# VictoriaMetrics/VictoriaLogs

Hardware: AMD Instinct MI355X
Metric: matched-rows/sec (higher is better)
Workload: dtype u8; 1 GPU; 100M rows, AND(phrase, re2 regex) on two string columns, 1xMI355X; rows_per_gpu=100000000, live_rows_per_gpu=100000000, msg_len=256, matched_rows_per_pass=100000000, parallelism=dp1

## Files before the change

### victorialogs_amd/csrc/core/regex.cpp

```cpp
#include "regex.h"

#include <cstring>

#include "match.h"
#include "tokenizer.h"
#include "unicode_case.h"

namespace vl {

namespace {

struct RNode {
  enum Kind {
    Lit, Dot, Concat, Alt, Star, Plus, Quest, Group, Empty, Class, Assert
  } kind;
  std::string lit;
  std::vector<RNode> subs;
  uint8_t cls[32] = {0};
  bool cls_nonascii = false;
  uint8_t assert_kind = 0;
};

static const uint32_t kFoldOrbits[][4] = {
    {0x004B, 0x006B, 0x212A, 0},
// ... 534 lines not shown
        out.push_back("");
        return true;
      }
      std::vector<std::string> prefixes;
      if (!get_or_values(n.subs[0], prefixes) || prefixes.empty()) return false;
      if (n.subs.size() == 1) {
        out = std::move(prefixes);
        return true;
      }
      RNode rest;
      rest.kind = RNode::Concat;
      rest.subs.assign(n.subs.begin() + 1, n.subs.end());
      std::vector<std::string> suffixes;
      if (!get_or_values(rest, suffixes) || suffixes.empty()) return false;
      if (prefixes.size() * suffixes.size() > kMaxOrValues) return false;
      for (const auto& p : prefixes) {
        for (const auto& q : suffixes) out.push_back(p + q);
      }
      return true;
    }
    default:
      return false;
  }
}

void collect_literals(const RNode& raw, std::vector<std::string>& out) {
  const RNode* n = &raw;
  while (n->kind == RNode::Group) n = &n->subs[0];
  if (n->kind == RNode::Lit) {
    out.push_back(n->lit);
    return;
  }
  if (n->kind != RNode::Concat) return;
  for (const auto& sub : n->subs) {
    const RNode* s = &sub;
    while (s->kind == RNode::Group) s = &s->subs[0];
    if (s->kind == RNode::Lit) out.push_back(s->lit);
  }
}



struct GAtom {
  uint8_t set[32];
};

struct PMask {
  uint64_t w0 = 0, w1 = 0;
  void set(int i) { (i < 64 ? w0 : w1) |= uint64_t(1) << (i & 63); }
  void operator|=(const PMask& o) {
    w0 |= o.w0;
    w1 |= o.w1;
  }
};

template <typename F>
static void pm_foreach(const PMask& m, F f) {
  uint64_t v = m.w0;
  while (v) {
    f(__builtin_ctzll(v));
    v &= v - 1;
  }
  v = m.w1;
  while (v) {
    f(64 + __builtin_ctzll(v));
    v &= v - 1;
  }
// ... 647 lines not shown
```

### victorialogs_amd/csrc/hip/scan_kernels.hip

```cpp
#include <hip/hip_runtime.h>

#include "../core/parse_float.h"
#include "../core/ryu.h"
#include "scan_types.h"

namespace vl {



__device__ int64_t g_vl_local_tz_nsecs = 0;

#include "scan_rowops.h"

typedef const __attribute__((address_space(3))) uint8_t* LdsBytePtr;

struct LdsTileAcc {
  LdsBytePtr tile;
  typedef const __attribute__((address_space(3))) uint64_t* LdsU64Ptr;
  __device__ __forceinline__ long swz(long off) const {
    return TileAcc{nullptr}.swz(off);
  }
  __device__ __forceinline__ uint64_t u64a(long off) const {
    return *(LdsU64Ptr)(tile + swz(off));
  }
  __device__ __forceinline__ void u64a2(long off, uint64_t* x0,
                                        uint64_t* x1) const {
    LdsU64Ptr p = (LdsU64Ptr)(tile + swz(off));
    *x0 = p[0];
    *x1 = p[1];
  }
  __device__ __forceinline__ uint8_t u8(long off) const { return tile[swz(off)]; }
};

__device__ __forceinline__ void d_fill_operand_slot(uint8_t* slot,
                                                    const uint8_t* src,
                                                    uint32_t n, int tid,
                                                    int bdim) {
  for (uint32_t k = tid; k < n; k += bdim) slot[k] = src[k];
}

extern "C" int vql_set_local_tz_nsecs(long long v) {
  int64_t x = v;
  return hipMemcpyToSymbol(HIP_SYMBOL(g_vl_local_tz_nsecs), &x, sizeof(x)) ==
                 hipSuccess
             ? 0
             : -1;
}
// ... 292 lines not shown
      o_next = col_offs[min(r0 + next_wd * 64 + uint32_t(lane), r1)];
      if (lane == 0) o_end_next = col_offs[min(r0 + next_wd * 64 + 64, r1)];
    }
    if (use_tile) {
      asm volatile("s_waitcnt lgkmcnt(0)" ::: "memory");
    }
    bool pred1 = false, pred2 = false;
    if (uint32_t(lane) < ng) {
      const long s = o_lane;
      const long e = uint32_t(__shfl(int(o_lane), lane + 1, 64));
      const long e_fix = uint32_t(lane) == ng - 1 ? long(byte1) : e;
      if (use_tile) {
        LdsTileAcc a{(LdsBytePtr)wtile};
        pred1 = d_match_phrase_at(a, s - byte0, e_fix - s, p1, n1, f1);
        pred2 = d_match_phrase_at(a, s - byte0, e_fix - s, p2, n2, f2);
      } else {
        GlobalAcc a{col_data};
        pred1 = d_match_phrase_at(a, s, e_fix - s, p1, n1, f1);
        pred2 = d_match_phrase_at(a, s, e_fix - s, p2, n2, f2);
      }
    }
    const uint64_t word1 = __ballot(pred1);
    const uint64_t word2 = __ballot(pred2);
    if (lane == 0) {
      out1[wd] = word1;
      out2[wd] = word2;
    }
    o_lane = o_next;
    o_end = o_end_next;
    wd = next_wd;
  }
}

__device__ __forceinline__ bool d_bloom_gate_ok(const DevLeafBlock& lb,
                                                int tid, int bdim,
                                                int* shared_flag) {
  if (!lb.nhashes) return true;
  __syncthreads();
  if (tid == 0) *shared_flag = 1;
  __syncthreads();
  if (lb.bloom_words > 0) {
    const uint64_t max_bits = uint64_t(lb.bloom_words) * 64;
    bool miss = false;
    for (uint32_t k = tid; k < lb.nhashes; k += bdim) {
      uint64_t idx = lb.hashes[k] % max_bits;
      if (((lb.bloom[idx >> 6] >> (idx & 63)) & 1) == 0) miss = true;
    }
    if (miss) *shared_flag = 0;
  }
  __syncthreads();
  return *shared_flag != 0;
}


__global__ __launch_bounds__(256) void scan_program_kernel(
    const DevOp* __restrict__ ops, int nops, const DevLeafBlock* __restrict__ lbs,
    int nleaves, const DevBlock* __restrict__ blocks,
    const DevChunk* __restrict__ chunks, unsigned long long* __restrict__ hits) {
  __shared__ uint64_t stack[kMaxStackDepth][kChunkWords];
  __shared__ __attribute__((aligned(16))) uint8_t tile[kNumWaves * kWaveTileBytes];
  __shared__ int bloom_ok;
  __shared__ unsigned long long wave_sums[4];
  __shared__ __attribute__((aligned(16))) uint8_t opnd[2][kOperandSlotBytes];

  const DevChunk ck = chunks[blockIdx.x];
  const DevBlock blk = blocks[ck.block];
  const uint32_t r0 = ck.chunk * kChunkRows;
  const uint32_t r1 = min(blk.rows, r0 + kChunkRows);
  const uint32_t nwords = (r1 - r0 + 63) / 64;
  const int tid = threadIdx.x;
  const int lane = tid & 63;
  const int wave = tid >> 6;
  const int nwaves = blockDim.x >> 6;
  const LdsBytePtr opnd0 = (LdsBytePtr)&opnd[0][0];
  const LdsBytePtr opnd1 = (LdsBytePtr)&opnd[1][0];

  int sp = 0;
  for (int i = 0; i < nops; i++) {
    const DevOp op = ops[i];
    __syncthreads();
    if (op.kind == kOpLeaf) {
      const DevLeafBlock& lb = lbs[size_t(ck.block) * nleaves + op.leaf];
      uint64_t* out = stack[sp];
      if (i + 1 < nops && ops[i + 1].kind == kOpLeaf &&
          lb.kind == kScanPhraseStr && lb.mode == kModeScan && lb.sg <= 1 &&
          sp + 1 < kMaxStackDepth) {
        const DevLeafBlock& lb2 =
            lbs[size_t(ck.block) * nleaves + ops[i + 1].leaf];
        if (lb2.kind == kScanPhraseStr && lb2.mode == kModeScan &&
            lb2.data == lb.data && lb2.offsets == lb.offsets &&
            lb.operand_len <= kOperandSlotBytes &&
            lb2.operand_len <= kOperandSlotBytes) {
          d_fill_operand_slot(opnd[0], lb.operand, lb.operand_len, tid,
                              blockDim.x);
          d_fill_operand_slot(opnd[1], lb2.operand, lb2.operand_len, tid,
                              blockDim.x);
          const bool ok1 = d_bloom_gate_ok(lb, tid, blockDim.x, &bloom_ok);
          const bool ok2 = d_bloom_gate_ok(lb2, tid, blockDim.x, &bloom_ok);
          __syncthreads();
          if (ok1 && ok2) {
            d_string_phrase2_loop(lb.data, lb.offsets,
                                  tile + wave * kWaveTileBytes, stack[sp],
                                  stack[sp + 1], r0, r1, nwords, lane, wave,
                                  nwaves, opnd0, lb.operand_len, lb.flags,
                                  opnd1, lb2.operand_len, lb2.flags);
            sp += 2;
            i++;
            continue;
          }
        }
      }
      if (lb.mode == kModeNone || lb.mode == kModeAll) {
        uint64_t fill = lb.mode == kModeAll ? ~uint64_t(0) : 0;
        for (uint32_t w = tid; w < nwords; w += blockDim.x) out[w] = fill;
        sp++;
        continue;
      }
      bool lds_phrase = false;
      uint32_t lds_len = 0;
      uint8_t lds_flags = 0;
      if (lb.kind == kScanPhraseStr) {
        if (lb.operand_len <= kOperandSlotBytes) {
          lds_phrase = true;
          lds_len = lb.operand_len;
          lds_flags = lb.flags;
          d_fill_operand_slot(opnd[0], lb.operand, lds_len, tid, blockDim.x);
        }
      } else if (lb.kind == kScanRegexStr) {
        const uint8_t* blob = lb.operand;
        const uint8_t re_flags = blob[0];
        if ((re_flags & kReOnlyPrefix) && !(re_flags & (kReNfa | kReAlways))) {
          const uint32_t plen = uint32_t(blob[1]) | uint32_t(blob[2]) << 8;
          if (plen >= 1 && plen <= kOperandSlotBytes) {
            lds_phrase = true;
            lds_len = plen;
            d_fill_operand_slot(opnd[0], blob + 7, plen, tid, blockDim.x);
          }
        }
      }
      if (!lb.nhashes) {
        if (lds_phrase) __syncthreads();
      } else {
        if (tid == 0) bloom_ok = 1;
        __syncthreads();
        if (lb.bloom_words > 0) {
          const uint64_t max_bits = uint64_t(lb.bloom_words) * 64;
          bool miss = false;
          for (uint32_t k = tid; k < lb.nhashes; k += blockDim.x) {
            uint64_t idx = lb.hashes[k] % max_bits;
            if (((lb.bloom[idx >> 6] >> (idx & 63)) & 1) == 0) miss = true;
          }
          if (miss) bloom_ok = 0;
        }
        __syncthreads();
        if (!bloom_ok) {
          for (uint32_t w = tid; w < nwords; w += blockDim.x) out[w] = 0;
          sp++;
          continue;
        }
      }

      if (d_is_string_kind(lb.kind)) {
        uint8_t* wtile = tile + wave * kWaveTileBytes;
        const uint8_t* col_data = lb.data;
        const uint32_t* col_offs = lb.offsets;
        const uint8_t* op_ptr = lb.operand;
        const uint32_t sgw = lb.sg;
        if (lds_phrase) {
          auto eval = [=](const auto& a, long s0, long sn) {
            return d_match_phrase_at(a, s0, sn, opnd0, lds_len, lds_flags);
          };
          if (sgw > 1) {
            d_string_smallrow_loop<false>(col_data, col_offs, nullptr, nullptr,
                                          wtile, out, r0, r1, nwords, sgw,
                                          lane, wave, nwaves, eval);
          } else {
            d_string_tile_loop<false>(col_data, col_offs, nullptr, nullptr,
                                      wtile, out, r0, r1, nwords, lane, wave,
                                      nwaves, eval);
          }
        } else if (lb.kind == kScanRegexStr) {
          auto eval = [=](const auto& a, long s0, long sn) {
            return d_regex_match_at(op_ptr, a, s0, sn);
          };
          if (sgw > 1) {
            d_string_smallrow_loop<false>(col_data, col_offs, nullptr, nullptr,
                                          wtile, out, r0, r1, nwords, sgw,
                                          lane, wave, nwaves, eval);
          } else {
            d_string_tile_loop<false>(col_data, col_offs, nullptr, nullptr,
                                      wtile, out, r0, r1, nwords, lane, wave,
                                      nwaves, eval);
          }
// ... 345 lines not shown
```

### victorialogs_amd/csrc/hip/scan_rowops.h

```cpp
#pragma once

#include "../core/unicode_ranges.inc"

extern __device__ int64_t g_vl_local_tz_nsecs;

__device__ __forceinline__ bool d_is_token_char(uint8_t c) {
  return (c >= 'a' && c <= 'z') || (c >= 'A' && c <= 'Z') ||
         (c >= '0' && c <= '9') || c == '_';
}

__device__ bool d_is_token_rune(uint32_t r) {
  if (r < 0x80) return d_is_token_char(uint8_t(r));
  int lo = 0, hi = kTokenRuneRangesCount - 1;
  while (lo <= hi) {
    int mid = (lo + hi) >> 1;
    if (r < kTokenRuneRanges[mid][0]) {
      hi = mid - 1;
    } else if (r > kTokenRuneRanges[mid][1]) {
      lo = mid + 1;
    } else {
      return true;
    }
  }
  return false;
// ... 72 lines not shown
  } else if ((c0 & 0xF8) == 0xF0) {
    len = 4; r = c0 & 0x07; lo = 0x10000;
  } else {
    return 0xFFFD;
  }
  if (len > n) return 0xFFFD;
  for (int i = 1; i < len; i++) {
    uint8_t c = a.u8(off + i);
    if ((c & 0xC0) != 0x80) return 0xFFFD;
    r = (r << 6) | (c & 0x3F);
  }
  if (r < lo || r > 0x10FFFF || (r >= 0xD800 && r <= 0xDFFF)) return 0xFFFD;
  *size = len;
  return r;
}

template <typename A>
__device__ uint32_t d_utf8_decode_last(const A& a, long off, long n, int* size) {
  *size = 1;
  if (n <= 0) return 0xFFFD;
  long start = n - 1;
  if (a.u8(off + start) < 0x80) return a.u8(off + start);
  long lim = n >= 4 ? n - 4 : 0;
  while (start > lim && (a.u8(off + start) & 0xC0) == 0x80) start--;
  int sz;
  uint32_t r = d_utf8_decode(a, off + start, n - start, &sz);
  if (start + sz != n) return 0xFFFD;
  *size = sz;
  return r;
}

__device__ __forceinline__ uint64_t d_swar_zero(uint64_t t) {
  return (t - 0x0101010101010101ULL) & ~t & 0x8080808080808080ULL;
}

template <typename A, typename P>
__device__ long d_index_at(const A& a, long s0, long sn, P sub, long subn) {
  if (subn == 0) return 0;
  if (subn > sn) return -1;
  const uint8_t c0 = sub[0];
  const uint64_t pat = 0x0101010101010101ULL * c0;
  const uint64_t pat1 = subn > 1 ? 0x0101010101010101ULL * sub[1] : 0;
  const long last = s0 + sn - subn;
  for (long w = s0 & ~15L; w <= last; w += 32) {
    uint64_t x0, x1, x2, x3;
    a.u64a2(w, &x0, &x1);
    a.u64a2(w + 16, &x2, &x3);
    uint64_t hitA = d_swar_zero(x0 ^ pat);
    uint64_t hitB = d_swar_zero(x1 ^ pat);
    uint64_t hitC = d_swar_zero(x2 ^ pat);
    uint64_t hitD = d_swar_zero(x3 ^ pat);
    if (subn > 1 && (hitA | hitB | hitC | hitD)) {
      const uint64_t h1A = d_swar_zero(x0 ^ pat1);
      const uint64_t h1B = d_swar_zero(x1 ^ pat1);
      const uint64_t h1C = d_swar_zero(x2 ^ pat1);
      const uint64_t h1D = d_swar_zero(x3 ^ pat1);
      hitA &= (h1A >> 8) | ((h1B & 0x80) << 56);
      hitB &= (h1B >> 8) | ((h1C & 0x80) << 56);
      hitC &= (h1C >> 8) | ((h1D & 0x80) << 56);
      hitD &= (h1D >> 8) | 0x8000000000000000ULL;
    }
    if (w < s0) {
      const long off = s0 - w;
      if (off >= 8) {
        hitA = 0;
        hitB &= ~((uint64_t(1) << ((off - 8) * 8)) - 1);
      } else {
        hitA &= ~((uint64_t(1) << (off * 8)) - 1);
      }
    }
    while (hitA | hitB | hitC | hitD) {
      long k;
      if (hitA) {
        k = long(__builtin_ctzll(hitA) >> 3);
        hitA &= hitA - 1;
      } else if (hitB) {
        k = 8 + long(__builtin_ctzll(hitB) >> 3);
        hitB &= hitB - 1;
      } else if (hitC) {
        k = 16 + long(__builtin_ctzll(hitC) >> 3);
        hitC &= hitC - 1;
      } else {
        k = 24 + long(__builtin_ctzll(hitD) >> 3);
        hitD &= hitD - 1;
      }
      const long pos = w + k;
      if (pos > last) return -1;
      bool eq = true;
      for (long i = 0; i < subn; i++) {
        if (a.u8(pos + i) != sub[i]) {
          eq = false;
          break;
        }
      }
      if (eq) return pos - s0;
    }
  }
  return -1;
}

template <typename A, typename P>
__device__ long d_get_phrase_pos_at(const A& a, long s0, long sn, P ph,
                                    long phn, uint8_t flags) {
  if (phn == 0) return 0;
  if (phn > sn) return -1;
  long pos = 0;
  for (;;) {
    long n = d_index_at(a, s0 + pos, sn - pos, ph, phn);
    if (n < 0) return -1;
    pos += n;
    if ((flags & kPhraseStartsToken) && pos > 0) {
      uint32_t rb = a.u8(s0 + pos - 1);
      if (rb >= 0x80) {
        int sz;
        rb = d_utf8_decode_last(a, s0, pos, &sz);
      }
      if (rb == 0xFFFD || d_is_token_rune(rb)) {
        pos++;
        continue;
      }
    }
    if ((flags & kPhraseEndsToken) && pos + phn < sn) {
      uint32_t ra = a.u8(s0 + pos + phn);
      if (ra >= 0x80) {
        int sz;
        ra = d_utf8_decode(a, s0 + pos + phn, sn - pos - phn, &sz);
      }
      if (ra == 0xFFFD || d_is_token_rune(ra)) {
// ... 1523 lines not shown
```

### victorialogs_amd/csrc/hip/scan_types.h

```cpp
#pragma once

#include <cstdint>

namespace vl {

constexpr uint32_t kChunkRows = 8192;
constexpr uint32_t kChunkWords = kChunkRows / 64;
constexpr uint32_t kWaveTileBytes = 17408;
constexpr uint32_t kNumWaves = 4;
constexpr uint32_t kOperandSlotBytes = 512;
constexpr int kMaxProgOps = 64;
constexpr int kMaxStackDepth = 8;

enum LeafMode : uint8_t {
  kModeNone = 0,
  kModeAll = 1,
  kModeScan = 2,
};

enum ScanKind : uint8_t {
  kScanPhraseStr = 0,
  kScanEqStr = 1,
  kScanEqBin = 2,
  kScanDict = 3,
// ... 39 lines not shown
  kScanLeFieldI64 = 43,
  kScanLeFieldF64 = 44,
  kScanLeFieldBinStr = 45,
  kScanEqFieldStr = 46,
  kScanLeFieldStr = 47,
};

enum : uint8_t {
  kFmtU64 = 1,
  kFmtI64 = 2,
  kFmtF64 = 3,
  kFmtIp = 4,
  kFmtIso = 5,
};

enum : uint8_t {
  kPhraseStartsToken = 1,
  kPhraseEndsToken = 2,
};

enum OpKind : uint8_t { kOpLeaf = 0, kOpAnd = 1, kOpOr = 2, kOpNot = 3 };

struct DevOp {
  uint8_t kind;
  uint8_t nargs;
  uint16_t leaf;
};

struct DevLeafBlock {
  uint8_t mode;
  uint8_t kind;
  uint8_t width;
  uint8_t flags;
  uint32_t nhashes;
  uint32_t bloom_words;
  uint32_t dict_mask;
  uint32_t operand_len;
  uint32_t sg;
  const uint64_t* hashes;
  const uint64_t* bloom;
  const uint8_t* operand;
  const uint8_t* data;
  const uint32_t* offsets;
  const int64_t* ts;
  uint64_t vmin, vmax;
};

struct DevBlock {
  uint64_t* bitmap_out;
  unsigned long long* hits_out;
  uint32_t rows;
  uint32_t pad;
};

struct DevChunk {
  uint32_t block;
  uint32_t chunk;
};

enum : uint8_t {
  kReOnlyPrefix = 1,
  kReDotStar = 2,
  kReDotPlus = 4,
  kReSubstrStar = 8,
  kReSubstrPlus = 16,
  kReHasOr = 32,
  kReNfa = 64,
  kReAlways = 128,
// ... 41 lines not shown
```

### victorialogs_amd/csrc/vql_api.cpp

```cpp
#include <hip/hip_runtime.h>

#include <algorithm>
#include <cmath>
#include <cstring>
#include <functional>
#include <map>
#include <memory>
#include <chrono>
#include <mutex>
#include <thread>
#include <string>
#include <vector>

#include "core/filter.h"
#include "core/bloom.h"
#include "core/match.h"
#include "core/op_serialize.h"
#include "core/tokenizer.h"
#include "core/unicode_case.h"
#include "core/part_reader.h"
#include "core/values.h"
#include "hip/scan_types.h"

namespace vl {
// ... 65 lines not shown
        return d;
      }
      case FilterNode::Not: {
        int d = flatten(n.children[0]);
        DevOp op;
        op.kind = kOpNot;
        op.nargs = 1;
        op.leaf = 0;
        ops.push_back(op);
        return d;
      }
      default: {
        DevOp op;
        op.kind = kOpLeaf;
        op.nargs = 0;
        op.leaf = uint16_t(leaves.size());
        leaves.push_back(&n);
        ops.push_back(op);
        return 1;
      }
    }
  }
};




struct LeafInfo {
  const FilterNode* node;
  std::string cname;
  bytes operand;
  uint8_t phrase_flags = 0;
  const uint8_t* d_operand = nullptr;
  const uint64_t* d_hashes = nullptr;
};

struct Stage {
  VqlPart* part;
  std::shared_ptr<VqlFilter> filter;
  int device = 0;
  long lo = 0, hi = 0;
  std::vector<std::pair<VqlPart*, long>> block_refs;

  static constexpr size_t kSlabBytes = size_t(256) << 20;
  static constexpr size_t kSlabTailPad = 4096;
  std::vector<std::pair<uint8_t*, size_t>> slabs;
  uint8_t* cur_slab = nullptr;
  size_t cur_cap = 0, cur_used = 0;

  DevOp* d_ops = nullptr;
  DevLeafBlock* d_lbs = nullptr;
  DevBlock* d_blocks = nullptr;
  DevChunk* d_chunks = nullptr;
  unsigned long long* d_hits = nullptr;
  unsigned long long* d_block_hits = nullptr;
  uint64_t* d_bitmap = nullptr;
  size_t bitmap_words = 0;
  uint32_t nchunks = 0;

  std::vector<uint64_t> block_word_off;
  uint64_t staged_bytes = 0;
  uint64_t algo_bytes = 0;
  uint64_t rows = 0;
  uint64_t live_rows = 0;

  std::vector<std::pair<uint64_t, uint64_t>> zero_word_ranges;
  bool bitmap_zeroed = false;
// ... 72 lines not shown
    staged_bytes = m.staged_bytes;
  }
};

struct StagedStrCol {
  bool is_const = false;
  std::string const_value;
  const uint8_t* d_data = nullptr;
  const uint32_t* d_offsets = nullptr;
  uint64_t data_bytes = 0;
  uint64_t rows = 0;
  uint32_t sg = 1;
};

static uint32_t pick_super_group(const std::vector<uint32_t>& offs,
                                 uint64_t rows) {
  if (rows == 0 || offs.size() < rows + 1) return 1;
  const uint64_t nwords = (rows + 63) / 64;
  for (uint32_t sg = 8; sg >= 2; sg /= 2) {
    const uint64_t nsg = (nwords + sg - 1) / sg;
    const uint64_t cap = std::max<uint64_t>(1, nsg / 32);
    uint64_t over = 0;
    for (uint64_t g = 0; g < nsg && over <= cap; g++) {
      const uint64_t ra = g * sg * 64;
      const uint64_t rb = std::min<uint64_t>(rows, ra + uint64_t(sg) * 64);
      const uint64_t span = uint64_t(offs[rb]) - (uint64_t(offs[ra]) & ~15ull);
      if (span > kWaveTileBytes) over++;
    }
    if (over <= cap) return sg;
  }
  return 1;
}

struct StagedBloom {
  const uint64_t* d_words = nullptr;
  uint32_t nwords = 0;
};

struct BlockStageCtx {
  Stage* st;
  const PartReader* pr;
  const BlockHeader* bh;
  PartReader::BlockColumns bc;
  std::map<std::string, StagedStrCol> cols;
  std::map<std::string, StagedBloom> blooms;
  std::map<std::string, std::vector<uint64_t>> host_blooms;
  const int64_t* d_ts = nullptr;

  const StagedStrCol& stage_column(const ColumnHeader& ch) {
    auto it = cols.find(ch.name);
    if (it != cols.end()) return it->second;
    StringsBlockDec dec;
    pr->read_values(ch, bh->rows_count, dec);
    StagedStrCol sc;
    sc.rows = bh->rows_count;
    if (dec.is_const) {
      sc.is_const = true;
      sc.const_value.assign((const char*)dec.data.data(), dec.data.size());
    } else {
      sc.d_data = st->push(dec.data.data(), dec.data.size());
      st->reserve(1024);
      sc.d_offsets = (const uint32_t*)st->push(dec.offsets.data(),
                                               dec.offsets.size() * 4, 4);
      sc.data_bytes = dec.data.size();
      sc.sg = pick_super_group(dec.offsets, sc.rows);
    }
    return cols.emplace(ch.name, std::move(sc)).first->second;
  }

  const std::vector<uint64_t>& bloom_host(const ColumnHeader& ch) {
    auto it = host_blooms.find(ch.name);
    if (it == host_blooms.end()) {
      std::vector<uint64_t> words;
      pr->read_bloom(ch, words);
      it = host_blooms.emplace(ch.name, std::move(words)).first;
    }
    return it->second;
  }

  const StagedBloom& stage_bloom(const ColumnHeader& ch) {
    auto it = blooms.find(ch.name);
    if (it != blooms.end()) return it->second;
    const std::vector<uint64_t>& words = bloom_host(ch);
    StagedBloom sb;
    sb.nwords = uint32_t(words.size());
    sb.d_words = (const uint64_t*)st->push(words.data(), words.size() * 8, 8);
    return blooms.emplace(ch.name, sb).first->second;
  }

  const int64_t* stage_timestamps() {
    if (!d_ts) {
      std::vector<int64_t> ts;
      pr->read_timestamps(*bh, ts);
      d_ts = (const int64_t*)st->push(ts.data(), ts.size() * 8, 8);
    }
    return d_ts;
  }
};

void set_bloom_gate(DevLeafBlock& lb, BlockStageCtx& ctx, const ColumnHeader& ch,
                    const LeafInfo& li) {
  const auto& hashes = li.node->token_hashes;
  if (hashes.empty()) return;
  const StagedBloom& sb = ctx.stage_bloom(ch);
  lb.nhashes = uint32_t(hashes.size());
  lb.hashes = li.d_hashes;
  lb.bloom = sb.d_words;
  lb.bloom_words = sb.nwords;
}

bool stage_eq_bin(DevLeafBlock& lb, BlockStageCtx& ctx, const ColumnHeader& ch,
                  const LeafInfo& li, Stage& st, const bytes& bin) {
  const StagedStrCol& sc = ctx.stage_column(ch);
  if (sc.is_const) {
    lb.mode = sc.const_value.size() == bin.size() &&
                      memcmp(sc.const_value.data(), bin.data(), bin.size()) == 0
                  ? kModeAll
                  : kModeNone;
    return false;
  }
  lb.mode = kModeScan;
  lb.kind = kScanEqBin;
  lb.width = uint8_t(bin.size());
  lb.operand = (const uint8_t*)st.push(bin.data(), bin.size(), 8);
  lb.operand_len = uint32_t(bin.size());
  lb.data = sc.d_data;
  set_bloom_gate(lb, ctx, ch, li);
  return true;
}

void stage_eq_bin_nogate(DevLeafBlock& lb, BlockStageCtx& ctx,
                         const ColumnHeader& ch, Stage& st, const bytes& bin) {
  const StagedStrCol& sc = ctx.stage_column(ch);
  if (sc.is_const) {
    lb.mode = sc.const_value.size() == bin.size() &&
                      memcmp(sc.const_value.data(), bin.data(), bin.size()) == 0
                  ? kModeAll
                  : kModeNone;
    return;
  }
  lb.mode = kModeScan;
  lb.kind = kScanEqBin;
  lb.width = uint8_t(bin.size());
  lb.operand = (const uint8_t*)st.push(bin.data(), bin.size(), 8);
  lb.operand_len = uint32_t(bin.size());
  lb.data = sc.d_data;
}

bool in_sorted_bin_host(const std::vector<std::string>& sorted_set, strview v) {
  size_t lo = 0, hi = sorted_set.size();
  while (lo < hi) {
    size_t mid = (lo + hi) / 2;
    const std::string& m = sorted_set[mid];
    int c = memcmp(m.data(), v.p, std::min(m.size(), v.n));
    if (c == 0) c = m.size() < v.n ? -1 : (m.size() > v.n ? 1 : 0);
    if (c == 0) return true;
    if (c < 0) {
      lo = mid + 1;
    } else {
      hi = mid;
    }
// ... 208 lines not shown
    case ValueType::TimestampISO8601: return "iso8601";
    default: return "unknown";
  }
}

uint8_t fmt_of_type(ValueType t) {
  switch (t) {
    case ValueType::Uint8:
    case ValueType::Uint16:
    case ValueType::Uint32:
    case ValueType::Uint64: return kFmtU64;
    case ValueType::Int64: return kFmtI64;
    case ValueType::Float64: return kFmtF64;
    case ValueType::IPv4: return kFmtIp;
    case ValueType::TimestampISO8601: return kFmtIso;
    default: return 0;
  }
}

uint8_t width_of_type(ValueType t) {
  switch (t) {
    case ValueType::Uint8: return 1;
    case ValueType::Uint16: return 2;
    case ValueType::Uint32: return 4;
    case ValueType::IPv4: return 4;
    default: return 8;
  }
}

void stage_leaf(const LeafInfo& li, BlockStageCtx& ctx, Stage& st, DevLeafBlock& lb) {
  const FilterNode& f = *li.node;
  const PartReader& pr = *ctx.pr;
  memset(&lb, 0, sizeof(lb));

  auto const_val = [&]() -> std::string {
    std::string v;
    if (!pr.get_const_column(ctx.bc, li.cname, &v)) return "";
    return v;
  };

  switch (f.type) {
    case FilterNode::Noop:
      lb.mode = kModeAll;
      return;

    case FilterNode::Time: {
      const TimestampsHeader& th = ctx.bh->timestamps_header;
      if (f.min_ts > f.max_ts || f.min_ts > th.max_timestamp ||
          f.max_ts < th.min_timestamp) {
        lb.mode = kModeNone;
        return;
      }
      if (f.min_ts <= th.min_timestamp && f.max_ts >= th.max_timestamp) {
        lb.mode = kModeAll;
        return;
      }
      lb.mode = kModeScan;
      lb.kind = kScanTsRange;
      lb.ts = ctx.stage_timestamps();
      lb.vmin = uint64_t(f.min_ts);
      lb.vmax = uint64_t(f.max_ts);
      return;
    }

    case FilterNode::Phrase: {
      strview phrase(f.phrase);
// ... 208 lines not shown
        return;
      }
      const StagedStrCol& sc = ctx.stage_column(ch);
      if (sc.is_const) {
        std::string s;
        strview v(sc.const_value);
        switch (ch.type) {
          case ValueType::String: s = sc.const_value; break;
          case ValueType::Uint8: format_uint64(s, uint8_t(v.p[0])); break;
          case ValueType::Uint16: format_uint64(s, get_u16be((const uint8_t*)v.p)); break;
          case ValueType::Uint32: format_uint64(s, get_u32be((const uint8_t*)v.p)); break;
          case ValueType::Uint64: format_uint64(s, get_u64be((const uint8_t*)v.p)); break;
          case ValueType::Int64: format_int64(s, get_i64be_zigzag((const uint8_t*)v.p)); break;
          case ValueType::Float64: {
            uint64_t u = get_u64be((const uint8_t*)v.p);
            double d;
            memcpy(&d, &u, 8);
            format_float64(s, d);
            break;
          }
          case ValueType::IPv4: format_ipv4(s, get_u32be((const uint8_t*)v.p)); break;
          case ValueType::TimestampISO8601:
            format_timestamp_iso8601(s, int64_t(get_u64be((const uint8_t*)v.p)));
            break;
          default: fail("unexpected const column type");
        }
        lb.mode = regex_match(f.re, strview(s)) ? kModeAll : kModeNone;
        return;
      }
      lb.mode = kModeScan;
      lb.operand = li.d_operand;
      lb.operand_len = uint32_t(li.operand.size());
      lb.data = sc.d_data;
      set_bloom_gate(lb, ctx, ch, li);
      switch (ch.type) {
        case ValueType::String:
          lb.kind = kScanRegexStr;
          lb.offsets = sc.d_offsets;
          return;
        case ValueType::Uint8: lb.kind = kScanRegexU; lb.width = 1; return;
        case ValueType::Uint16: lb.kind = kScanRegexU; lb.width = 2; return;
        case ValueType::Uint32: lb.kind = kScanRegexU; lb.width = 4; return;
        case ValueType::Uint64: lb.kind = kScanRegexU; lb.width = 8; return;
        case ValueType::Int64: lb.kind = kScanRegexI; lb.width = 8; return;
        case ValueType::Float64: lb.kind = kScanRegexF64; lb.width = 8; return;
        case ValueType::IPv4: lb.kind = kScanRegexIp; lb.width = 4; return;
        case ValueType::TimestampISO8601: lb.kind = kScanRegexIso; lb.width = 8; return;
        default: fail("unknown valueType while staging regexp filter");
      }
    }

    case FilterNode::Range: {
      double min_v = f.min_f, max_v = f.max_f;
      if (min_v > max_v) {
        lb.mode = kModeNone;
        return;
      }
      std::string cv = const_val();
      if (!cv.empty()) {
        double x = parse_math_number(strview(cv));
        lb.mode = (x >= min_v && x <= max_v) ? kModeAll : kModeNone;
        return;
      }
      ColumnHeader ch;
      if (!pr.get_column_header(ctx.bc, li.cname, &ch)) {
        lb.mode = kModeNone;
        return;
      }
      if (ch.type == ValueType::Dict) {
        uint32_t mask = dict_mask_of(ch.dict, [&](strview dv) {
          double x = parse_math_number(dv);
          return x >= min_v && x <= max_v;
        });
        stage_dict(lb, ctx, ch, mask);
        return;
      }
      if (ch.type == ValueType::String) {
        const StagedStrCol& sc = ctx.stage_column(ch);
        if (sc.is_const) {
          double x = parse_math_number(strview(sc.const_value));
          lb.mode = (x >= min_v && x <= max_v) ? kModeAll : kModeNone;
          return;
// ... 460 lines not shown
          return;
        }
        case ValueType::Float64: {
          const StagedStrCol& sc = ctx.stage_column(ch);
          if (sc.is_const) {
            std::string str = format_encoded(ch.type, strview(sc.const_value));
            lb.mode = match_sequence(strview(str), phrases) ? kModeAll
                                                            : kModeNone;
            return;
          }
          lb.mode = kModeScan;
          lb.kind = kScanSeqFmt;
          lb.width = 8;
          lb.flags = uint8_t(kFmtF64 << 4);
          lb.operand = li.d_operand;
          lb.operand_len = uint32_t(li.operand.size());
          lb.data = sc.d_data;
          set_bloom_gate(lb, ctx, ch, li);
          return;
        }
        case ValueType::IPv4:
        case ValueType::TimestampISO8601: {
          if (phrases.size() == 1) {
            FilterNode tmp;
            tmp.type = FilterNode::Phrase;
            tmp.field = f.field;
            tmp.phrase = phrases[0];
            tmp.token_hashes = f.token_hashes;
            LeafInfo tmp_li;
            tmp_li.node = &tmp;
            tmp_li.cname = li.cname;
            tmp_li.operand.assign(phrases[0].begin(), phrases[0].end());
            tmp_li.phrase_flags = phrase_flags_of(phrases[0]);
            tmp_li.d_hashes = li.d_hashes;
            tmp_li.d_operand =
                (const uint8_t*)st.push(tmp_li.operand.data(),
                                        tmp_li.operand.size(), 8);
            stage_leaf(tmp_li, ctx, st, lb);
            return;
          }
          const StagedStrCol& sc = ctx.stage_column(ch);
          if (sc.is_const) {
            std::string str = format_encoded(ch.type, strview(sc.const_value));
            lb.mode = match_sequence(strview(str), phrases) ? kModeAll
                                                            : kModeNone;
            return;
          }
          lb.mode = kModeScan;
          lb.kind = kScanSeqFmt;
          lb.width = ch.type == ValueType::IPv4 ? 4 : 8;
          lb.flags = uint8_t((ch.type == ValueType::IPv4 ? kFmtIp : kFmtIso) << 4);
          lb.operand = li.d_operand;
          lb.operand_len = uint32_t(li.operand.size());
          lb.data = sc.d_data;
          set_bloom_gate(lb, ctx, ch, li);
          return;
        }
        default:
          fail("unknown valueType while staging sequence filter");
      }
    }


    case FilterNode::In: {
      if (f.values.empty()) {
        lb.mode = kModeNone;
        return;
// ... 585 lines not shown
          lb.mode = kModeScan;
          lb.kind = is_ph ? kScanAnyCasePhraseStr : kScanAnyCasePrefixStr;
          lb.flags = li.phrase_flags;
          lb.operand = li.d_operand;
          lb.operand_len = uint32_t(f.min_s.size());
          lb.data = sc.d_data;
          lb.offsets = sc.d_offsets;
          if (any) {
            lb.hashes = (const uint64_t*)st.push(mask.data(), nw * 8, 8);
            lb.bloom = (const uint64_t*)st.push(val.data(), nw * 8, 8);
          }
          return;
        }
        case ValueType::Dict: {
          uint32_t m = dict_mask_of(ch.dict, host_match);
          stage_dict(lb, ctx, ch, m);
          return;
        }
        default: {
          const bool iso = ch.type == ValueType::TimestampISO8601;
          FilterNode tmp;
          tmp.type = is_ph ? FilterNode::Phrase : FilterNode::Prefix;
          tmp.field = f.field;
          tmp.phrase = iso ? f.max_s : f.min_s;
          tmp.token_hashes = iso ? f.all_hashes : f.token_hashes;
          LeafInfo tmp_li;
          tmp_li.node = &tmp;
          tmp_li.cname = li.cname;
          tmp_li.operand.assign(tmp.phrase.begin(), tmp.phrase.end());
          tmp_li.phrase_flags = phrase_flags_of(tmp.phrase);
          if (!tmp_li.operand.empty()) {
            tmp_li.d_operand = (const uint8_t*)st.push(tmp_li.operand.data(),
                                                       tmp_li.operand.size(), 8);
          }
          if (!tmp.token_hashes.empty()) {
            tmp_li.d_hashes = (const uint64_t*)st.push(
                tmp.token_hashes.data(), tmp.token_hashes.size() * 8, 8);
          }
          stage_leaf(tmp_li, ctx, st, lb);
          return;
        }
      }
    }


    case FilterNode::EqField:
    case FilterNode::LeField: {
      const bool is_le = f.type == FilterNode::LeField;
      const bool excl = is_le && f.min_u != 0;
      const std::string other = canonical_field(f.min_s);
      if (li.cname == other) {
        lb.mode = excl ? kModeNone : kModeAll;
        return;
      }
      std::string cva, cvb;
      bool a_const = pr.get_const_column(ctx.bc, li.cname, &cva) && !cva.empty();
      bool b_const = pr.get_const_column(ctx.bc, other, &cvb) && !cvb.empty();
      ColumnHeader cha, chb;
      bool a_col = !a_const && pr.get_column_header(ctx.bc, li.cname, &cha);
      bool b_col = !b_const && pr.get_column_header(ctx.bc, other, &chb);
      if (a_const && b_const) {
        bool m = is_le ? le_values_string(strview(cva), strview(cvb), excl)
                       : cva == cvb;
        lb.mode = m ? kModeAll : kModeNone;
        return;
      }
      if (!a_const && !a_col && !b_const && !b_col) {
        lb.mode = excl ? kModeNone : kModeAll;
        return;
      }
// ... 218 lines not shown
        bytes b;
        auto put32 = [&](uint32_t v) {
          b.push_back(uint8_t(v));
          b.push_back(uint8_t(v >> 8));
          b.push_back(uint8_t(v >> 16));
          b.push_back(uint8_t(v >> 24));
        };
        put32(uint32_t(li.node->min_s.size()));
        put32(uint32_t(li.node->max_s.size()));
        b.insert(b.end(), li.node->min_s.begin(), li.node->min_s.end());
        b.insert(b.end(), li.node->max_s.begin(), li.node->max_s.end());
        li.operand = std::move(b);
        break;
      }
      case FilterNode::DayRange:
      case FilterNode::WeekRange: {
        bytes b(8);
        int64_t off = li.node->tz_offset;
        memcpy(b.data(), &off, 8);
        li.operand = std::move(b);
        break;
      }
      case FilterNode::AnyCasePhrase:
      case FilterNode::AnyCasePrefix:
        li.operand.assign(li.node->min_s.begin(), li.node->min_s.end());
        li.phrase_flags = phrase_flags_of(li.node->min_s);
        break;
      default:
        break;
    }
    if (!li.operand.empty()) {
      li.d_operand = st->push(li.operand.data(), li.operand.size(), 8);
    }
    if (!li.node->token_hashes.empty()) {
      li.d_hashes = (const uint64_t*)st->push(li.node->token_hashes.data(),
                                              li.node->token_hashes.size() * 8, 8);
    }
  }

  st->block_word_off.resize(size_t(nblocks) + 1, 0);
  for (long b = 0; b < nblocks; b++) {
    st->block_word_off[size_t(b) + 1] =
        st->block_word_off[size_t(b)] + (bh_of(b).rows_count + 63) / 64;
  }
  st->bitmap_words = size_t(st->block_word_off.back());
  st->d_bitmap = (uint64_t*)st->reserve(st->bitmap_words * 8, 8);

  std::vector<DevBlock> blocks_h((size_t(nblocks)));
  std::vector<DevLeafBlock> lbs_h(size_t(nblocks) * size_t(nleaves));
  std::vector<DevChunk> chunks_h;
  for (long b = 0; b < nblocks; b++) {
    VqlPart* bp = st->block_refs[size_t(b)].first;
    const BlockHeader& bh = bh_of(b);
    BlockStageCtx ctx;
    ctx.st = st.get();
    ctx.pr = &bp->pr;
    ctx.bh = &bh;
    bp->pr.read_block_columns(bh, ctx.bc);

    DevBlock& db = blocks_h[size_t(b)];
    db.rows = uint32_t(bh.rows_count);
    db.bitmap_out = st->d_bitmap + st->block_word_off[size_t(b)];
    db.hits_out = nullptr;

    const Stage::ArenaMark arena_mark = st->mark();
    uint64_t block_algo = 0;

    for (int l = 0; l < nleaves; l++) {
      DevLeafBlock& lb = lbs_h[size_t(b) * size_t(nleaves) + size_t(l)];
      stage_leaf(leaf_infos[size_t(l)], ctx, *st, lb);
// ... 590 lines not shown
```

Measured before the change: 17.48 billion rows/s.

## Move bloom gate to host, group substring verify, merge adjacent regex literals

Bloom-filter gating moves from the kernel, which used extra barriers and global hash loads per leaf, to host staging. A block whose bloom check fails now becomes a kModeNone leaf, and its freshly staged column upload is rolled back. Substring verification compares bytes in fixed groups of 4 (or 8) using 32-bit LDS operand loads instead of a byte-by-byte early-exit loop. Regex literal collection also concatenates adjacent literal nodes into longer required substrings. Together these remove kernel synchronisation and per-byte compare branching, at the cost of host-side bloom work and a more complex staging arena.

Result: faster. 18.55 billion rows/s (median of 6 runs) (+6.1%).

```diff
diff --git a/victorialogs_amd/csrc/core/regex.cpp b/victorialogs_amd/csrc/core/regex.cpp
--- a/victorialogs_amd/csrc/core/regex.cpp
+++ b/victorialogs_amd/csrc/core/regex.cpp
@@ -590,7 +590,18 @@
     return;
   }
   if (n->kind != RNode::Concat) return;
+  bool run = false;
   for (const auto& sub : n->subs) {
+    if (sub.kind == RNode::Lit) {
+      if (run) {
+        out.back() += sub.lit;
+      } else {
+        out.push_back(sub.lit);
+      }
+      run = true;
+      continue;
+    }
+    run = false;
     const RNode* s = &sub;
     while (s->kind == RNode::Group) s = &s->subs[0];
     if (s->kind == RNode::Lit) out.push_back(s->lit);
diff --git a/victorialogs_amd/csrc/hip/scan_kernels.hip b/victorialogs_amd/csrc/hip/scan_kernels.hip
--- a/victorialogs_amd/csrc/hip/scan_kernels.hip
+++ b/victorialogs_amd/csrc/hip/scan_kernels.hip
@@ -10,9 +10,13 @@
 
 __device__ int64_t g_vl_local_tz_nsecs = 0;
 
+typedef const __attribute__((address_space(3))) uint8_t* LdsBytePtr;
+
+__device__ __forceinline__ uint32_t d_operand4(LdsBytePtr sub, long i) {
+  return *(const __attribute__((address_space(3))) uint32_t*)(sub + i);
+}
+
 #include "scan_rowops.h"
-
-typedef const __attribute__((address_space(3))) uint8_t* LdsBytePtr;
 
 struct LdsTileAcc {
   LdsBytePtr tile;
@@ -371,26 +375,6 @@
   }
 }
 
-__device__ __forceinline__ bool d_bloom_gate_ok(const DevLeafBlock& lb,
-                                                int tid, int bdim,
-                                                int* shared_flag) {
-  if (!lb.nhashes) return true;
-  __syncthreads();
-  if (tid == 0) *shared_flag = 1;
-  __syncthreads();
-  if (lb.bloom_words > 0) {
-    const uint64_t max_bits = uint64_t(lb.bloom_words) * 64;
-    bool miss = false;
-    for (uint32_t k = tid; k < lb.nhashes; k += bdim) {
-      uint64_t idx = lb.hashes[k] % max_bits;
-      if (((lb.bloom[idx >> 6] >> (idx & 63)) & 1) == 0) miss = true;
-    }
-    if (miss) *shared_flag = 0;
-  }
-  __syncthreads();
-  return *shared_flag != 0;
-}
-
 
 __global__ __launch_bounds__(256) void scan_program_kernel(
     const DevOp* __restrict__ ops, int nops, const DevLeafBlock* __restrict__ lbs,
@@ -398,7 +382,6 @@
     const DevChunk* __restrict__ chunks, unsigned long long* __restrict__ hits) {
   __shared__ uint64_t stack[kMaxStackDepth][kChunkWords];
   __shared__ __attribute__((aligned(16))) uint8_t tile[kNumWaves * kWaveTileBytes];
-  __shared__ int bloom_ok;
   __shared__ unsigned long long wave_sums[4];
   __shared__ __attribute__((aligned(16))) uint8_t opnd[2][kOperandSlotBytes];
 
@@ -434,19 +417,15 @@
                               blockDim.x);
           d_fill_operand_slot(opnd[1], lb2.operand, lb2.operand_len, tid,
                               blockDim.x);
-          const bool ok1 = d_bloom_gate_ok(lb, tid, blockDim.x, &bloom_ok);
-          const bool ok2 = d_bloom_gate_ok(lb2, tid, blockDim.x, &bloom_ok);
           __syncthreads();
-          if (ok1 && ok2) {
-            d_string_phrase2_loop(lb.data, lb.offsets,
-                                  tile + wave * kWaveTileBytes, stack[sp],
-                                  stack[sp + 1], r0, r1, nwords, lane, wave,
-                                  nwaves, opnd0, lb.operand_len, lb.flags,
-                                  opnd1, lb2.operand_len, lb2.flags);
-            sp += 2;
-            i++;
-            continue;
-          }
+          d_string_phrase2_loop(lb.data, lb.offsets,
+                                tile + wave * kWaveTileBytes, stack[sp],
+                                stack[sp + 1], r0, r1, nwords, lane, wave,
+                                nwaves, opnd0, lb.operand_len, lb.flags,
+                                opnd1, lb2.operand_len, lb2.flags);
+          sp += 2;
+          i++;
+          continue;
         }
       }
       if (lb.mode == kModeNone || lb.mode == kModeAll) {
@@ -477,27 +456,7 @@
           }
         }
       }
-      if (!lb.nhashes) {
-        if (lds_phrase) __syncthreads();
-      } else {
-        if (tid == 0) bloom_ok = 1;
-        __syncthreads();
-        if (lb.bloom_words > 0) {
-          const uint64_t max_bits = uint64_t(lb.bloom_words) * 64;
-          bool miss = false;
-          for (uint32_t k = tid; k < lb.nhashes; k += blockDim.x) {
-            uint64_t idx = lb.hashes[k] % max_bits;
-            if (((lb.bloom[idx >> 6] >> (idx & 63)) & 1) == 0) miss = true;
-          }
-          if (miss) bloom_ok = 0;
-        }
-        __syncthreads();
-        if (!bloom_ok) {
-          for (uint32_t w = tid; w < nwords; w += blockDim.x) out[w] = 0;
-          sp++;
-          continue;
-        }
-      }
+      if (lds_phrase) __syncthreads();
 
       if (d_is_string_kind(lb.kind)) {
         uint8_t* wtile = tile + wave * kWaveTileBytes;
diff --git a/victorialogs_amd/csrc/hip/scan_rowops.h b/victorialogs_amd/csrc/hip/scan_rowops.h
--- a/victorialogs_amd/csrc/hip/scan_rowops.h
+++ b/victorialogs_amd/csrc/hip/scan_rowops.h
@@ -128,6 +128,45 @@
 
 __device__ __forceinline__ uint64_t d_swar_zero(uint64_t t) {
   return (t - 0x0101010101010101ULL) & ~t & 0x8080808080808080ULL;
+}
+
+#ifndef VL_VERIFY_GROUP
+#define VL_VERIFY_GROUP 4
+#endif
+constexpr int kVerifyGroup = VL_VERIFY_GROUP;
+static_assert(kVerifyGroup == 4 || kVerifyGroup == 8, "verify group width");
+
+template <typename P>
+__device__ __forceinline__ uint32_t d_operand4(P sub, long i) {
+  return uint32_t(sub[i]) | uint32_t(sub[i + 1]) << 8 |
+         uint32_t(sub[i + 2]) << 16 | uint32_t(sub[i + 3]) << 24;
+}
+
+template <typename A, typename P>
+__device__ __forceinline__ bool d_verify_at(const A& a, long pos, P sub,
+                                            long subn) {
+  long i = 0;
+  for (; i + kVerifyGroup <= subn; i += kVerifyGroup) {
+    uint32_t diff = 0;
+    for (int g = 0; g < kVerifyGroup; g += 4) {
+      const uint32_t t = uint32_t(a.u8(pos + i + g)) |
+                         uint32_t(a.u8(pos + i + g + 1)) << 8 |
+                         uint32_t(a.u8(pos + i + g + 2)) << 16 |
+                         uint32_t(a.u8(pos + i + g + 3)) << 24;
+      diff |= t ^ d_operand4(sub, i + g);
+    }
+    if (diff) return false;
+  }
+  const long rem = subn - i;
+  if (rem > 0) {
+    uint32_t diff = 0;
+    for (int k = 0; k < kVerifyGroup - 1; k++) {
+      const long j = i + (k < rem ? k : rem - 1);
+      diff |= uint32_t(a.u8(pos + j)) ^ uint32_t(sub[j]);
+    }
+    if (diff) return false;
+  }
+  return true;
 }
 
 template <typename A, typename P>
@@ -182,14 +221,7 @@
       }
       const long pos = w + k;
       if (pos > last) return -1;
-      bool eq = true;
-      for (long i = 0; i < subn; i++) {
-        if (a.u8(pos + i) != sub[i]) {
-          eq = false;
-          break;
-        }
-      }
-      if (eq) return pos - s0;
+      if (d_verify_at(a, pos, sub, subn)) return pos - s0;
     }
   }
   return -1;
diff --git a/victorialogs_amd/csrc/hip/scan_types.h b/victorialogs_amd/csrc/hip/scan_types.h
--- a/victorialogs_amd/csrc/hip/scan_types.h
+++ b/victorialogs_amd/csrc/hip/scan_types.h
@@ -95,8 +95,7 @@
   uint8_t kind;
   uint8_t width;
   uint8_t flags;
-  uint32_t nhashes;
-  uint32_t bloom_words;
+  uint32_t pad_[2];
   uint32_t dict_mask;
   uint32_t operand_len;
   uint32_t sg;
diff --git a/victorialogs_amd/csrc/vql_api.cpp b/victorialogs_amd/csrc/vql_api.cpp
--- a/victorialogs_amd/csrc/vql_api.cpp
+++ b/victorialogs_amd/csrc/vql_api.cpp
@@ -121,7 +121,6 @@
   bytes operand;
   uint8_t phrase_flags = 0;
   const uint8_t* d_operand = nullptr;
-  const uint64_t* d_hashes = nullptr;
 };
 
 struct Stage {
@@ -260,20 +259,17 @@
   return 1;
 }
 
-struct StagedBloom {
-  const uint64_t* d_words = nullptr;
-  uint32_t nwords = 0;
-};
-
 struct BlockStageCtx {
   Stage* st;
   const PartReader* pr;
   const BlockHeader* bh;
   PartReader::BlockColumns bc;
   std::map<std::string, StagedStrCol> cols;
-  std::map<std::string, StagedBloom> blooms;
   std::map<std::string, std::vector<uint64_t>> host_blooms;
   const int64_t* d_ts = nullptr;
+  bool has_fresh = false;
+  std::string fresh_col;
+  Stage::ArenaMark fresh_mark{};
 
   const StagedStrCol& stage_column(const ColumnHeader& ch) {
     auto it = cols.find(ch.name);
@@ -286,6 +282,9 @@
       sc.is_const = true;
       sc.const_value.assign((const char*)dec.data.data(), dec.data.size());
     } else {
+      has_fresh = true;
+      fresh_col = ch.name;
+      fresh_mark = st->mark();
       sc.d_data = st->push(dec.data.data(), dec.data.size());
       st->reserve(1024);
       sc.d_offsets = (const uint32_t*)st->push(dec.offsets.data(),
@@ -306,16 +305,6 @@
     return it->second;
   }
 
-  const StagedBloom& stage_bloom(const ColumnHeader& ch) {
-    auto it = blooms.find(ch.name);
-    if (it != blooms.end()) return it->second;
-    const std::vector<uint64_t>& words = bloom_host(ch);
-    StagedBloom sb;
-    sb.nwords = uint32_t(words.size());
-    sb.d_words = (const uint64_t*)st->push(words.data(), words.size() * 8, 8);
-    return blooms.emplace(ch.name, sb).first->second;
-  }
-
   const int64_t* stage_timestamps() {
     if (!d_ts) {
       std::vector<int64_t> ts;
@@ -326,15 +315,19 @@
   }
 };
 
+bool h_bloom_all(BlockStageCtx& ctx, const ColumnHeader& ch,
+                 const std::vector<uint64_t>& hashes);
+
 void set_bloom_gate(DevLeafBlock& lb, BlockStageCtx& ctx, const ColumnHeader& ch,
                     const LeafInfo& li) {
-  const auto& hashes = li.node->token_hashes;
-  if (hashes.empty()) return;
-  const StagedBloom& sb = ctx.stage_bloom(ch);
-  lb.nhashes = uint32_t(hashes.size());
-  lb.hashes = li.d_hashes;
-  lb.bloom = sb.d_words;
-  lb.bloom_words = sb.nwords;
+  if (h_bloom_all(ctx, ch, li.node->token_hashes)) return;
+  lb = DevLeafBlock{};
+  lb.mode = kModeNone;
+  if (ctx.has_fresh && ctx.fresh_col == ch.name) {
+    ctx.st->rollback(ctx.fresh_mark);
+    ctx.cols.erase(ch.name);
+    ctx.has_fresh = false;
+  }
 }
 
 bool stage_eq_bin(DevLeafBlock& lb, BlockStageCtx& ctx, const ColumnHeader& ch,
@@ -354,7 +347,7 @@
   lb.operand_len = uint32_t(bin.size());
   lb.data = sc.d_data;
   set_bloom_gate(lb, ctx, ch, li);
-  return true;
+  return lb.mode == kModeScan;
 }
 
 void stage_eq_bin_nogate(DevLeafBlock& lb, BlockStageCtx& ctx,
@@ -629,6 +622,7 @@
   const FilterNode& f = *li.node;
   const PartReader& pr = *ctx.pr;
   memset(&lb, 0, sizeof(lb));
+  ctx.has_fresh = false;
 
   auto const_val = [&]() -> std::string {
     std::string v;
@@ -903,22 +897,23 @@
       lb.operand = li.d_operand;
       lb.operand_len = uint32_t(li.operand.size());
       lb.data = sc.d_data;
-      set_bloom_gate(lb, ctx, ch, li);
       switch (ch.type) {
         case ValueType::String:
           lb.kind = kScanRegexStr;
           lb.offsets = sc.d_offsets;
-          return;
-        case ValueType::Uint8: lb.kind = kScanRegexU; lb.width = 1; return;
-        case ValueType::Uint16: lb.kind = kScanRegexU; lb.width = 2; return;
-        case ValueType::Uint32: lb.kind = kScanRegexU; lb.width = 4; return;
-        case ValueType::Uint64: lb.kind = kScanRegexU; lb.width = 8; return;
-        case ValueType::Int64: lb.kind = kScanRegexI; lb.width = 8; return;
-        case ValueType::Float64: lb.kind = kScanRegexF64; lb.width = 8; return;
-        case ValueType::IPv4: lb.kind = kScanRegexIp; lb.width = 4; return;
-        case ValueType::TimestampISO8601: lb.kind = kScanRegexIso; lb.width = 8; return;
+          break;
+        case ValueType::Uint8: lb.kind = kScanRegexU; lb.width = 1; break;
+        case ValueType::Uint16: lb.kind = kScanRegexU; lb.width = 2; break;
+        case ValueType::Uint32: lb.kind = kScanRegexU; lb.width = 4; break;
+        case ValueType::Uint64: lb.kind = kScanRegexU; lb.width = 8; break;
+        case ValueType::Int64: lb.kind = kScanRegexI; lb.width = 8; break;
+        case ValueType::Float64: lb.kind = kScanRegexF64; lb.width = 8; break;
+        case ValueType::IPv4: lb.kind = kScanRegexIp; lb.width = 4; break;
+        case ValueType::TimestampISO8601: lb.kind = kScanRegexIso; lb.width = 8; break;
         default: fail("unknown valueType while staging regexp filter");
       }
+      set_bloom_gate(lb, ctx, ch, li);
+      return;
     }
 
     case FilterNode::Range: {
@@ -1445,7 +1440,6 @@
             tmp_li.cname = li.cname;
             tmp_li.operand.assign(phrases[0].begin(), phrases[0].end());
             tmp_li.phrase_flags = phrase_flags_of(phrases[0]);
-            tmp_li.d_hashes = li.d_hashes;
             tmp_li.d_operand =
                 (const uint8_t*)st.push(tmp_li.operand.data(),
                                         tmp_li.operand.size(), 8);
@@ -2097,10 +2091,6 @@
           if (!tmp_li.operand.empty()) {
             tmp_li.d_operand = (const uint8_t*)st.push(tmp_li.operand.data(),
                                                        tmp_li.operand.size(), 8);
-          }
-          if (!tmp.token_hashes.empty()) {
-            tmp_li.d_hashes = (const uint64_t*)st.push(
-                tmp.token_hashes.data(), tmp.token_hashes.size() * 8, 8);
           }
           stage_leaf(tmp_li, ctx, st, lb);
           return;
@@ -2385,10 +2375,6 @@
     if (!li.operand.empty()) {
       li.d_operand = st->push(li.operand.data(), li.operand.size(), 8);
     }
-    if (!li.node->token_hashes.empty()) {
-      li.d_hashes = (const uint64_t*)st->push(li.node->token_hashes.data(),
-                                              li.node->token_hashes.size() * 8, 8);
-    }
   }
 
   st->block_word_off.resize(size_t(nblocks) + 1, 0);
```
